# wpeebles/gangealing

Measured on NVIDIA H100. Metric: gangealing_train_images_per_sec_256, higher is better.
Workload: dtype f32

## Files before the change

### gangealing_b200/csrc/nhwc.cu

```cuda
#include <cuda.h>

#include "common.cuh"
#include "nhwc_reduce.cuh"

namespace gg {
namespace {

constexpr int kT = 256;

template <typename T>
__global__ void __launch_bounds__(kT)
noise_bias_act_nhwc_kernel(T* __restrict__ out, const T* __restrict__ x, const float* __restrict__ noise,
                           const float* __restrict__ noise_weight, const float* __restrict__ bias,
                           const float* __restrict__ row_scale, float alpha, float gain, int64_t n_vec, int cv,
                           int64_t hw) {
  constexpr int V = ChanVec<T>::V;
  const float nw = noise ? (noise_weight ? __ldg(noise_weight) : 1.f) : 0.f;
  const int64_t base = (static_cast<int64_t>(blockIdx.x) * 4) * kT + threadIdx.x;
  uint4 xv[4];
#pragma unroll
  for (int u = 0; u < 4; ++u) {
    const int64_t v = base + static_cast<int64_t>(u) * kT;
    if (v < n_vec) xv[u] = ldg_stream16(x + v * V);
  }
// ... 285 lines not shown
  const int rows_out = min(p.seg_rows, p.out_h - oy0);
  const int x_out0 = bx * BX;
  const int c0 = cc * CB;
  const int iy0 = oy0 - p.pad_y0, ix0 = x_out0 - p.pad_x0;
  const int rows_in = rows_out + 3;
  const int n_stage_iters = (rows_in + kRY - 1) / kRY;
  constexpr uint32_t kStageBytes = G::STAGE_ELEMS * sizeof(T);

  if (tid == 0) {
#pragma unroll
    for (int s = 0; s < kNS; ++s) mbar_init(&full_bar[s], 1);
    mbar_fence_init();
  }
  __syncthreads();
  if (tid == 0) {
#pragma unroll
    for (int s = 0; s < kNS - 1; ++s)
      if (s < n_stage_iters) {
        mbar_expect_tx(&full_bar[s], kStageBytes);
        tma_load_4d(tiles + s * G::STAGE_ELEMS, &tmap, c0, ix0, iy0 + s * kRY, n, &full_bar[s]);
      }
  }

  float kf[4][4];
#pragma unroll
  for (int a = 0; a < 4; ++a)
#pragma unroll
    for (int b = 0; b < 4; ++b)
      kf[a][b] = (a < kh && b < kw) ? __ldg(filt + (kh - 1 - a) * kw + (kw - 1 - b)) : 0.f;
  float ku[4], kv[4];
  {
    int a0 = 0, b0 = 0;
    float big = 0.f;
#pragma unroll
    for (int a = 0; a < 4; ++a)
#pragma unroll
      for (int b = 0; b < 4; ++b)
        if (fabsf(kf[a][b]) > big) { big = fabsf(kf[a][b]); a0 = a; b0 = b; }
    float piv = 1.f;
#pragma unroll
    for (int a = 0; a < 4; ++a)
#pragma unroll
      for (int b = 0; b < 4; ++b)
        if (a == a0 && b == b0) piv = kf[a][b];
    const float inv = big > 0.f ? 1.f / piv : 0.f;
#pragma unroll
    for (int a = 0; a < 4; ++a) {
      float col = 0.f;
#pragma unroll
      for (int b = 0; b < 4; ++b) if (b == b0) col = kf[a][b];
      ku[a] = col * inv;
    }
#pragma unroll
    for (int b = 0; b < 4; ++b) {
      float row = 0.f;
#pragma unroll
      for (int a = 0; a < 4; ++a) if (a == a0) row = kf[a][b];
      kv[b] = row;
    }
  }

  float bq[V], rq[V], sq[V], dacc[V];
#pragma unroll
  for (int k = 0; k < V; ++k) { bq[k] = 0.f; rq[k] = 1.f; sq[k] = 1.f; dacc[k] = 0.f; }
  float nw = 0.f;
  const int64_t nc0 = static_cast<int64_t>(n) * p.c + c0 + cq * V;
  if (MODE != 0) {
    if (row_scale) {
#pragma unroll
      for (int k = 0; k < V; ++k) rq[k] = __ldg(row_scale + nc0 + k);
    }
  }
  if (FUSED) {
    if (bias) {
#pragma unroll
      for (int k = 0; k < V; ++k) bq[k] = __ldg(bias + c0 + cq * V + k);
    }
    if (scale2) {
#pragma unroll
      for (int k = 0; k < V; ++k) sq[k] = __ldg(scale2 + nc0 + k);
    }
    nw = noise ? (noise_weight ? __ldg(noise_weight) : 1.f) : 0.f;
  }
  constexpr bool fast = FUSED && FAST;
  const float neg = (p.act == 3) ? p.alpha : 1.f;
  if (fast) {
#pragma unroll
    for (int k = 0; k < V; ++k) { rq[k] *= p.gain; bq[k] *= p.gain; }
    nw *= p.gain;
  }
  const int xo = x_out0 + COLS * xg;
  const int64_t row_stride = static_cast<int64_t>(p.out_w) * p.c;
  const int64_t obase = ((static_cast<int64_t>(n) * p.out_h + oy0) * p.out_w + xo) * p.c + c0 + cq * V;
  int64_t ocur = obase - 3 * row_stride;
  bool okc[COLS];
#pragma unroll
  for (int j = 0; j < COLS; ++j) okc[j] = xo + j < p.out_w;
  float nzn[kRY][COLS];
#pragma unroll
  for (int rr = 0; rr < kRY; ++rr)
#pragma unroll
    for (int j = 0; j < COLS; ++j) nzn[rr][j] = 0.f;
  const float* noise_base = noise ? noise + (static_cast<int64_t>(n) * p.out_h + oy0) * p.out_w + xo : nullptr;
  auto fetch_noise = [&](int it_) {
#pragma unroll
    for (int rr = 0; rr < kRY; ++rr) {
      const int ro = it_ * kRY + rr - 3;
#pragma unroll
      for (int j = 0; j < COLS; ++j) nzn[rr][j] = 0.f;
      if (ro >= 0 && ro < rows_out) {
        const float* np_ = noise_base + static_cast<int64_t>(ro) * p.out_w;
#pragma unroll
        for (int j = 0; j < COLS; ++j)
          if (okc[j]) nzn[rr][j] = __ldg(np_ + j);
      }
    }
  };
  if (FUSED && noise) fetch_noise(0);

  uint4 mcur[COLS], mnext[COLS];
#pragma unroll
  for (int j = 0; j < COLS; ++j) mcur[j] = mnext[j] = make_uint4(0u, 0u, 0u, 0u);
  auto fetch_mul = [&](int ro_) {
    if (ro_ >= 0 && ro_ < rows_out) {
      const int64_t mo = obase + ro_ * row_stride;
#pragma unroll
      for (int j = 0; j < COLS; ++j)
        if (okc[j]) mnext[j] = __ldg(reinterpret_cast<const uint4*>(mul + mo + static_cast<int64_t>(j) * p.c));
    }
  };
  if (MODE == 2 && mul) { fetch_mul(-3 + 3); }

  float hwin[SEP ? 4 : 1][COLS][V];
  float rwin[SEP ? 1 : 4][COLS + 3][V];
  int r_in = 0;
  for (int it = 0; it < n_stage_iters; ++it) {
    const int stage = it % kNS;
    if (tid == 0) {
      const int nxt = it + kNS - 1;
      if (nxt < n_stage_iters) {
        const int ns = nxt % kNS;
        asm volatile("fence.proxy.async.shared::cta;" ::: "memory");
        mbar_expect_tx(&full_bar[ns], kStageBytes);
        tma_load_4d(tiles + ns * G::STAGE_ELEMS, &tmap, c0, ix0, iy0 + nxt * kRY, n, &full_bar[ns]);
      }
    }
    float nzc[kRY][COLS];
#pragma unroll
    for (int rr = 0; rr < kRY; ++rr)
#pragma unroll
      for (int j = 0; j < COLS; ++j) nzc[rr][j] = nzn[rr][j];
    if (FUSED && noise && it + 1 < n_stage_iters) fetch_noise(it + 1);
    if (MODE == 2 && mul && it + 1 < n_stage_iters) {
#pragma unroll
      for (int rr = 0; rr < kRY; ++rr) {
        const int ro = (it + 1) * kRY + rr - 3;
        if (ro >= 0 && ro < rows_out) {
          const T* mp = mul + obase + ro * row_stride;
#pragma unroll
          for (int j = 0; j < COLS; ++j)
            if (okc[j]) asm volatile("prefetch.global.L2 [%0];" ::"l"(mp + static_cast<int64_t>(j) * p.c));
        }
      }
    }
    mbar_wait(&full_bar[stage], static_cast<uint32_t>((it / kNS) & 1));
    const T* st = tiles + stage * G::STAGE_ELEMS;
#pragma unroll
    for (int rr = 0; rr < kRY; ++rr, ++r_in, ocur += row_stride) {
      if (MODE == 2 && mul) {
#pragma unroll
        for (int j = 0; j < COLS; ++j) mcur[j] = mnext[j];
        fetch_mul(r_in - 3 + 1);
      }
      const uint4* rowp = reinterpret_cast<const uint4*>(st + (rr * TW + COLS * xg) * CB) + cq;
      float q[COLS + 3][V];
#pragma unroll
      for (int i = 0; i < COLS + 3; ++i) ChanVec<T>::unpack(rowp[i * 8], q[i]);
      if constexpr (SEP) {
#pragma unroll
        for (int j = 0; j < COLS; ++j)
#pragma unroll
          for (int k = 0; k < V; ++k) {
            float h = __fmul_rn(kv[0], q[j][k]);
            h = __fmaf_rn(kv[1], q[j + 1][k], h);
            h = __fmaf_rn(kv[2], q[j + 2][k], h);
            h = __fmaf_rn(kv[3], q[j + 3][k], h);
            hwin[rr][j][k] = h;
          }
      } else {
#pragma unroll
        for (int i = 0; i < COLS + 3; ++i)
#pragma unroll
          for (int k = 0; k < V; ++k) rwin[rr][i][k] = q[i][k];
      }
      const int ro = r_in - 3;
      if (ro >= 0 && ro < rows_out) {
#pragma unroll
        for (int j = 0; j < COLS; ++j) {
          float a4[V];
          if constexpr (SEP) {
#pragma unroll
            for (int k = 0; k < V; ++k) {
              float a = __fmul_rn(ku[0], hwin[(rr + 1) & 3][j][k]);
              a = __fmaf_rn(ku[1], hwin[(rr + 2) & 3][j][k], a);
              a = __fmaf_rn(ku[2], hwin[(rr + 3) & 3][j][k], a);
              a = __fmaf_rn(ku[3], hwin[rr][j][k], a);
              a4[k] = a;
            }
          } else {
#pragma unroll
            for (int k = 0; k < V; ++k) a4[k] = 0.f;
#pragma unroll
            for (int a = 0; a < 4; ++a)
#pragma unroll
              for (int b = 0; b < 4; ++b)
#pragma unroll
                for (int k = 0; k < V; ++k) a4[k] = fmaf(kf[a][b], rwin[(rr + 1 + a) & 3][j + b][k], a4[k]);
          }
          const int64_t ooff = ocur + j * p.c;
          if (FUSED) {
            const float nzj = nw * nzc[rr][j];
            float o2[V];
#pragma unroll
            for (int k = 0; k < V; ++k) {
              float t = __fmaf_rn(a4[k], rq[k], __fadd_rn(bq[k], nzj));
              const float tn = __fmul_rn(t, neg);
              if (fast) t = fmaxf(t, tn);
              else t = (t > 0.f ? t : tn) * p.gain;
              a4[k] = t;
              o2[k] = __fmul_rn(t, sq[k]);
            }
            if (okc[j]) {
              if (out) *reinterpret_cast<uint4*>(out + ooff) = ChanVec<T>::pack(a4);
              if (out2) *reinterpret_cast<uint4*>(out2 + ooff) = ChanVec<T>::pack(o2);
            }
          } else if (MODE == 2) {
            if (okc[j]) {
              if (mul) {
                float mf[V];
                ChanVec<T>::unpack(mcur[j], mf);
#pragma unroll
                for (int k = 0; k < V; ++k) dacc[k] = fmaf(a4[k], mf[k], dacc[k]);
              }
#pragma unroll
              for (int k = 0; k < V; ++k) a4[k] *= rq[k];
              *reinterpret_cast<uint4*>(out + ooff) = ChanVec<T>::pack(a4);
            }
          } else {
            if (okc[j]) *reinterpret_cast<uint4*>(out + ooff) = ChanVec<T>::pack(a4);
          }
        }
      }
    }
    __syncthreads();
  }
  if (MODE == 2 && partial) {
    float* red = reinterpret_cast<float*>(tiles_raw);
#pragma unroll
    for (int k = 0; k < V; ++k) red[xg * CB + cq * V + k] = dacc[k];
    __syncthreads();
    if (tid < CB) {
      float t = 0.f;
#pragma unroll 8
      for (int g = 0; g < 32; ++g) t += red[g * CB + tid];
      const int64_t K = static_cast<int64_t>(gridDim.x / chunks) * gridDim.y;
      const int64_t kidx = static_cast<int64_t>(bx) * gridDim.y + blockIdx.y;
      partial[(static_cast<int64_t>(n) * K + kidx) * p.c + c0 + tid] = t;
    }
  }
}

typedef CUresult (*EncodeTiledFn)(CUtensorMap*, CUtensorMapDataType, cuuint32_t, void*, const cuuint64_t*, const cuuint64_t*,
                                  const cuuint32_t*, const cuuint32_t*, CUtensorMapInterleave, CUtensorMapSwizzle,
                                  CUtensorMapL2promotion, CUtensorMapFloatOOBfill);

inline EncodeTiledFn encode_fn() {
  static EncodeTiledFn fn = nullptr;
  if (!fn) {
    void* p = nullptr;
    cudaDriverEntryPointQueryResult q;
    if (cudaGetDriverEntryPoint("cuTensorMapEncodeTiled", &p, cudaEnableDefault, &q) == cudaSuccess &&
        q == cudaDriverEntryPointSuccess)
      fn = reinterpret_cast<EncodeTiledFn>(p);
  }
  return fn;
}

inline int grid1(int64_t total, int per_cta) {
  int64_t g = (total + per_cta - 1) / per_cta;
  return static_cast<int>(g > 0 ? g : 1);
}

}
}

using namespace gg;

extern "C" {

#define GG_DISPATCH_T(dtype_, who_, ...)                                                                   \
  switch (dtype_) {                                                                                        \
    case GG_F32: { using T_ = float; __VA_ARGS__; break; }                                                 \
    case GG_BF16: { using T_ = __nv_bfloat16; __VA_ARGS__; break; }                                        \
    default: return fail(GG_ERR_UNSUPPORTED, "%s: dtype %d not supported (fp32 or bf16)", who_, dtype_);  \
  }

static inline int vec_of(int dtype) { return dtype == GG_BF16 ? 8 : 4; }

int gg_noise_bias_act_nhwc(void* out, const void* x, const float* noise, const float* noise_weight, const float* bias,
                           const float* row_scale, int dtype, float alpha, float scale, int64_t N, int C, int64_t HW,
                           void* stream) {
  if (N < 0 || C < 0 || HW < 0) return fail(GG_ERR_BAD_ARG, "noise_bias_act_nhwc: negative size");
  if (dtype != GG_F32 && dtype != GG_BF16) return fail(GG_ERR_UNSUPPORTED, "noise_bias_act_nhwc: dtype %d not supported", dtype);
  const int64_t numel = N * HW * C;
  if (numel == 0) return GG_OK;
  const int V = vec_of(dtype);
  if (C % V != 0) return fail(GG_ERR_UNSUPPORTED, "noise_bias_act_nhwc: C must be a multiple of %d", V);
  if (!out || !x) return fail(GG_ERR_BAD_ARG, "noise_bias_act_nhwc: null tensor");
  const int64_t n_vec = numel / V;
  const int64_t grid = (n_vec + 4 * kT - 1) / (4 * kT);
  if (grid > 0x7fffffffLL) return fail(GG_ERR_BAD_ARG, "noise_bias_act_nhwc: tensor too large");
// ... 130 lines not shown

struct BlurPlan {
  int out_h, out_w, xblocks, chunks, segs, seg_rows;
};
static int blur_plan(BlurPlan* pl, int dtype, int64_t N, int C, int in_h, int in_w, int kernel_h, int kernel_w, int pad_x0,
                     int pad_x1, int pad_y0, int pad_y1) {
  const int V = vec_of(dtype);
  const int CB = 8 * V, BX = (V == 4) ? 64 : 32;
  if (C % CB != 0) return fail(GG_ERR_UNSUPPORTED, "blur_nhwc: C must be a multiple of %d", CB);
  pl->out_h = in_h + pad_y0 + pad_y1 - kernel_h + 1;
  pl->out_w = in_w + pad_x0 + pad_x1 - kernel_w + 1;
  if (pl->out_h < 1 || pl->out_w < 1) return fail(GG_ERR_BAD_ARG, "blur_nhwc: empty output");
  pl->xblocks = (pl->out_w + BX - 1) / BX;
  pl->chunks = C / CB;
  const int64_t base_ctas = static_cast<int64_t>(pl->xblocks) * pl->chunks * (N > 0 ? N : 1);
  int segs = static_cast<int>((2LL * 2 * sm_count() + base_ctas - 1) / base_ctas);
  int seg_rows = (pl->out_h + segs - 1) / segs;
  if (seg_rows < 16) seg_rows = pl->out_h < 16 ? pl->out_h : 16;
  seg_rows = (seg_rows + 3) / 4 * 4;
  pl->seg_rows = seg_rows;
  pl->segs = (pl->out_h + seg_rows - 1) / seg_rows;
  return GG_OK;
}

int64_t gg_blur_nhwc_workspace(int dtype, int64_t N, int C, int in_h, int in_w, int kernel_h, int kernel_w, int pad_x0,
                               int pad_x1, int pad_y0, int pad_y1) {
  BlurPlan pl;
  if (N <= 0 || C <= 0 || (dtype != GG_F32 && dtype != GG_BF16)) return 0;
  if (blur_plan(&pl, dtype, N, C, in_h, in_w, kernel_h, kernel_w, pad_x0, pad_x1, pad_y0, pad_y1) != GG_OK) return 0;
  return N * static_cast<int64_t>(pl.xblocks) * pl.segs * C * static_cast<int64_t>(sizeof(float));
}

}

template <typename T>
static int launch_blur(void* out, void* out2, const void* in, const float* kernel, const float* noise,
                       const float* noise_weight, const float* bias, const float* row_scale, const float* scale2,
                       const void* mul, float* row_dot, void* workspace, int64_t N, int C, int in_h, int in_w, int kernel_h,
                       int kernel_w, int separable, int pad_x0, int pad_x1, int pad_y0, int pad_y1, int mode, int act,
                       float alpha, float scale, void* stream, int dtype) {
  using G = BlurGeom<T>;
  BlurPlan pl;
  int rc = blur_plan(&pl, dtype, N, C, in_h, in_w, kernel_h, kernel_w, pad_x0, pad_x1, pad_y0, pad_y1);
  if (rc != GG_OK) return rc;
  EncodeTiledFn enc = encode_fn();
  if (!enc) return fail(GG_ERR_CUDA, "blur_nhwc: cuTensorMapEncodeTiled is not available from this driver");
  struct MapKey { const void* ptr; int64_t n; int c, h, w, es; };
  struct MapEnt { MapKey key; CUtensorMap map; bool valid; };
  static thread_local MapEnt cache[16] = {};
  static thread_local unsigned cache_next = 0;
  const MapKey key = {in, N, C, in_h, in_w, static_cast<int>(sizeof(T))};
  const CUtensorMap* cached = nullptr;
  for (int i = 0; i < 16 && !cached; ++i)
    if (cache[i].valid && cache[i].key.ptr == key.ptr && cache[i].key.n == key.n && cache[i].key.c == key.c &&
        cache[i].key.h == key.h && cache[i].key.w == key.w && cache[i].key.es == key.es)
      cached = &cache[i].map;
  CUtensorMap tmap;
  if (cached) tmap = *cached;
  const cuuint64_t es = sizeof(T);
  const cuuint64_t gdim[4] = {static_cast<cuuint64_t>(C), static_cast<cuuint64_t>(in_w), static_cast<cuuint64_t>(in_h),
                              static_cast<cuuint64_t>(N)};
  const cuuint64_t gstr[3] = {static_cast<cuuint64_t>(C) * es, static_cast<cuuint64_t>(in_w) * C * es,
                              static_cast<cuuint64_t>(in_h) * in_w * C * es};
  const cuuint32_t box[4] = {G::CB, G::TW, kRY, 1};
  const cuuint32_t estr[4] = {1, 1, 1, 1};
  if (!cached) {
    const CUresult r = enc(&tmap, sizeof(T) == 4 ? CU_TENSOR_MAP_DATA_TYPE_FLOAT32 : CU_TENSOR_MAP_DATA_TYPE_BFLOAT16, 4,
                           const_cast<void*>(in), gdim, gstr, box, estr, CU_TENSOR_MAP_INTERLEAVE_NONE,
                           CU_TENSOR_MAP_SWIZZLE_NONE, CU_TENSOR_MAP_L2_PROMOTION_L2_128B, CU_TENSOR_MAP_FLOAT_OOB_FILL_NONE);
    if (r != CUDA_SUCCESS) return fail(GG_ERR_CUDA, "blur_nhwc: cuTensorMapEncodeTiled failed (%d)", static_cast<int>(r));
    MapEnt& e = cache[cache_next++ % 16];
    e.key = key; e.map = tmap; e.valid = true;
  }
  BlurNhwcParams p;
  p.n = static_cast<int>(N); p.c = C; p.in_h = in_h; p.in_w = in_w; p.out_h = pl.out_h; p.out_w = pl.out_w;
  p.pad_x0 = pad_x0; p.pad_y0 = pad_y0;
  p.act = act; p.alpha = alpha; p.gain = scale;
  p.seg_rows = pl.seg_rows;
  const dim3 grid(static_cast<unsigned>(pl.xblocks * pl.chunks), static_cast<unsigned>(pl.segs), static_cast<unsigned>(N));
  const size_t smem = static_cast<size_t>(kNS) * G::STAGE_ELEMS * sizeof(T);
  static DeviceOnce configured;
  if (configured.needed()) {
    cudaError_t e = cudaSuccess;
    const void* kernels[8] = {reinterpret_cast<const void*>(blur_nhwc_kernel<T, 0, true>),
                              reinterpret_cast<const void*>(blur_nhwc_kernel<T, 0, false>),
                              reinterpret_cast<const void*>(blur_nhwc_kernel<T, 1, true, false>),
                              reinterpret_cast<const void*>(blur_nhwc_kernel<T, 1, false, false>),
                              reinterpret_cast<const void*>(blur_nhwc_kernel<T, 1, true, true>),
                              reinterpret_cast<const void*>(blur_nhwc_kernel<T, 1, false, true>),
                              reinterpret_cast<const void*>(blur_nhwc_kernel<T, 2, true>),
                              reinterpret_cast<const void*>(blur_nhwc_kernel<T, 2, false>)};
    for (int i = 0; i < 8 && e == cudaSuccess; ++i)
      e = cudaFuncSetAttribute(kernels[i], cudaFuncAttributeMaxDynamicSharedMemorySize, static_cast<int>(smem));
    if (e != cudaSuccess) return cuda_fail(e, "blur_nhwc smem opt-in");
    configured.done();
  }
  auto st = static_cast<cudaStream_t>(stream);
  float* partial = (mode == 2 && row_dot) ? static_cast<float*>(workspace) : nullptr;
  const bool fast = scale > 0.f && ((act == 3 && alpha >= 0.f && alpha <= 1.f) || act == 1);
#define GG_BLUR(M_, S_, F_)                                                                                          \
  blur_nhwc_kernel<T, M_, S_, F_><<<grid, kT, smem, st>>>(static_cast<T*>(out), static_cast<T*>(out2), tmap, kernel, kernel_h, \
                                                         kernel_w, noise, noise_weight, bias, row_scale, scale2,     \
                                                         static_cast<const T*>(mul), partial, p)
  if (mode == 1) {
    if (fast) { if (separable) GG_BLUR(1, true, true); else GG_BLUR(1, false, true); }
    else { if (separable) GG_BLUR(1, true, false); else GG_BLUR(1, false, false); }
  }
  else if (mode == 2) { if (separable) GG_BLUR(2, true, false); else GG_BLUR(2, false, false); }
  else { if (separable) GG_BLUR(0, true, false); else GG_BLUR(0, false, false); }
#undef GG_BLUR
  GG_CHECK_LAUNCH("blur_nhwc launch");
  if (partial) {
    const int K = pl.xblocks * pl.segs;
    nhwc_finish_kernel<<<static_cast<unsigned>(N * ((C + 31) / 32)), dim3(32, 32), 0, st>>>(row_dot, partial, N, K, C);
    GG_CHECK_LAUNCH("blur_nhwc finish launch");
  }
  return GG_OK;
}

extern "C" {

int gg_blur_nhwc(void* out, void* out2, const void* in, const float* kernel, const float* noise, const float* noise_weight,
                 const float* bias, const float* row_scale, const float* scale2, const void* mul, float* row_dot,
                 void* workspace, int dtype, int64_t N, int C, int in_h, int in_w, int kernel_h, int kernel_w, int separable,
                 int pad_x0, int pad_x1, int pad_y0, int pad_y1, int mode, int act, float alpha, float scale, void* stream) {
  if (N < 0 || C < 0 || in_h < 1 || in_w < 1) return fail(GG_ERR_BAD_ARG, "blur_nhwc: bad shape");
  if (kernel_h < 1 || kernel_w < 1 || kernel_h > 4 || kernel_w > 4) return fail(GG_ERR_UNSUPPORTED, "blur_nhwc: filter must be <= 4x4");
  if (mode < 0 || mode > 2) return fail(GG_ERR_BAD_ARG, "blur_nhwc: mode must be 0 (blur), 1 (fused tail) or 2 (adjoint epilogue)");
  if (act != 1 && act != 3) return fail(GG_ERR_UNSUPPORTED, "blur_nhwc: act must be 1 or 3");
  if (dtype != GG_F32 && dtype != GG_BF16) return fail(GG_ERR_UNSUPPORTED, "blur_nhwc: dtype %d not supported (fp32 or bf16)", dtype);
  if (N == 0 || C == 0) return GG_OK;
  if (!in || !kernel) return fail(GG_ERR_BAD_ARG, "blur_nhwc: null tensor");
  if (mode == 1 ? (!out && !out2) : !out) return fail(GG_ERR_BAD_ARG, "blur_nhwc: null output");
  if (mode != 1 && out2) return fail(GG_ERR_BAD_ARG, "blur_nhwc: out2 belongs to the fused tail (mode 1)");
  if (mode == 2 && row_dot && (!mul || !workspace)) return fail(GG_ERR_BAD_ARG, "blur_nhwc: row_dot needs `mul` and a workspace");
  if (N > 65535) return fail(GG_ERR_UNSUPPORTED, "blur_nhwc: batch > 65535");
  if (mode == 0) { noise = nullptr; noise_weight = nullptr; bias = nullptr; row_scale = nullptr; scale2 = nullptr; }
  GG_DISPATCH_T(dtype, "blur_nhwc",
                return launch_blur<T_>(out, out2, in, kernel, noise, noise_weight, bias, row_scale, scale2, mul, row_dot,
                                       workspace, N, C, in_h, in_w, kernel_h, kernel_w, separable, pad_x0, pad_x1, pad_y0,
                                       pad_y1, mode, act, alpha, scale, stream, dtype));
  return GG_OK;
}

}
```

### gangealing_b200/op/nhwc.py

```python
import torch

from .. import _lib

CL = torch.channels_last

TIMING = None


def blur_multiple(t):
    return 8 * _lib.nhwc_vec(t)


def _f32(t, numel=None):
    if t is None:
        return None
    t = t.detach()
    if t.dtype != torch.float32 or not t.is_contiguous():
        t = t.float().contiguous()
    if numel is not None and t.numel() != numel:
        raise RuntimeError("channels-last op: expected %d fp32 values, got %d" % (numel, t.numel()))
    return t


def noise_plane(noise, n, h, w):
    if noise is None:
        return None
    noise = noise.detach()
    if noise.numel() != n * h * w:
        noise = noise.expand(n, 1, h, w)
    return noise.float().contiguous()


def blur(x, kernel, pad, mode=0, noise=None, noise_weight=None, bias=None, row_scale=None, scale2=None, want_out=True,
         want_out2=False, mul=None, want_dot=False, negative_slope=0.2, gain=1.0, act=3):
    n, c, in_h, in_w = x.shape
    taps = kernel.detach()
    if taps.dtype != torch.float32 or not taps.is_contiguous():
        taps = taps.float().contiguous()
    kh, kw = taps.shape
    out_h = in_h + pad[2] + pad[3] - kh + 1
    out_w = in_w + pad[0] + pad[1] - kw + 1
    if out_h < 1 or out_w < 1:
        raise RuntimeError("blur: empty output (%d x %d)" % (out_h, out_w))
    lib = _lib.load()
    code = _lib.dtype_code(x)

    def empty():
        return torch.empty((n, c, out_h, out_w), dtype=x.dtype, device=x.device, memory_format=CL)
    out = empty() if (want_out or mode != 1) else None
    out2 = empty() if (mode == 1 and want_out2) else None
    nz = noise_plane(noise, n, out_h, out_w) if mode == 1 else None
    dot = ws = None
    if mode == 2 and want_dot:
        if mul is None or mul.shape != (n, c, out_h, out_w) or mul.dtype != x.dtype or not mul.is_contiguous(memory_format=CL):
            raise RuntimeError("blur (adjoint epilogue): `mul` must be a channels-last tensor of the output's shape and dtype")
        dot = torch.empty((n, c), dtype=torch.float32, device=x.device)
        nbytes = lib.gg_blur_nhwc_workspace(code, n, c, in_h, in_w, kh, kw, pad[0], pad[1], pad[2], pad[3])
        ws = torch.empty(max(1, nbytes // 4), dtype=torch.float32, device=x.device)
    timed = TIMING is not None and mode == 1
    if timed:
        ev0, ev1 = torch.cuda.Event(enable_timing=True), torch.cuda.Event(enable_timing=True)
        ev0.record()
    rc = lib.gg_blur_nhwc(_lib.ptr(out), _lib.ptr(out2), x.data_ptr(), taps.data_ptr(), _lib.ptr(nz),
                          _lib.ptr(_f32(noise_weight, 1)), _lib.ptr(_f32(bias, c)), _lib.ptr(_f32(row_scale, n * c)),
                          _lib.ptr(_f32(scale2, n * c)), _lib.ptr(mul if dot is not None else None), _lib.ptr(dot), _lib.ptr(ws),
                          code, n, c, in_h, in_w, kh, kw, 1 if _lib.filter_is_separable(kernel) else 0, pad[0], pad[1],
                          pad[2], pad[3], mode, act, negative_slope, gain, _lib.stream())
    _lib.check(rc, "gg_blur_nhwc")
    if timed:
        ev1.record()
        es = x.element_size()
        writes = (out is not None) + (out2 is not None)
        TIMING.append((ev0, ev1, es * n * c * (in_h * in_w + writes * out_h * out_w) + (4 * n * out_h * out_w if nz is not None else 0)
                       + 4 * ((2 + (scale2 is not None)) * c + 1 + kh * kw)))
    return out, out2, dot


def noise_bias_act(x, noise, noise_weight, bias, row_scale, negative_slope, gain):
    n, c, h, w = x.shape
    out = torch.empty_like(x)
    rc = _lib.load().gg_noise_bias_act_nhwc(out.data_ptr(), x.data_ptr(), _lib.ptr(noise_plane(noise, n, h, w)),
                                            _lib.ptr(_f32(noise_weight, 1)), _lib.ptr(_f32(bias, c)),
                                            _lib.ptr(_f32(row_scale, n * c)), _lib.dtype_code(x), negative_slope, gain,
                                            n, c, h * w, _lib.stream())
    _lib.check(rc, "gg_noise_bias_act_nhwc")
    return out


def bias_act_backward(g, out_saved, negative_slope, gain, want_bias_grad):
    n, c, h, w = out_saved.shape
    lib = _lib.load()
    gx = torch.empty_like(out_saved)
    grad_bias = ws = None
    if want_bias_grad:
        grad_bias = torch.empty(c, dtype=torch.float32, device=g.device)
        ws = torch.empty(max(1, lib.gg_nhwc_rowwise_workspace(n, c, h * w) // 4), dtype=torch.float32, device=g.device)
    rc = lib.gg_bias_act_backward_nhwc(gx.data_ptr(), _lib.ptr(grad_bias), _lib.ptr(ws), g.data_ptr(), out_saved.data_ptr(),
                                       _lib.dtype_code(out_saved), negative_slope, gain, n, c, h * w, _lib.stream())
    _lib.check(rc, "gg_bias_act_backward_nhwc")
    return gx, grad_bias


def channel_scale(x, s, y=None):
    n, c, h, w = x.shape
    lib = _lib.load()
    out = torch.empty_like(x)
    dot = ws = None
    if y is not None:
        dot = torch.empty((n, c), dtype=torch.float32, device=x.device)
        ws = torch.empty(max(1, lib.gg_nhwc_rowwise_workspace(n, c, h * w) // 4), dtype=torch.float32, device=x.device)
    rc = lib.gg_channel_scale_nhwc(out.data_ptr(), _lib.ptr(dot), _lib.ptr(ws), x.data_ptr(), _lib.ptr(y), _f32(s, n * c).data_ptr(),
                                   _lib.dtype_code(x), n, c, h * w, _lib.stream())
    _lib.check(rc, "gg_channel_scale_nhwc")
    return out, dot


def styled_tail(raw, noise, noise_weight, bias, demod, s_next, wm, rgb_bias, skip, want_out, negative_slope, gain, act=3):
    n, c, h, w = raw.shape
    out = torch.empty_like(raw) if want_out else None
    xs = torch.empty_like(raw) if s_next is not None else None
    rgb = torch.empty((n, 3, h, w), dtype=torch.float32, device=raw.device) if wm is not None else None
    sk = None
    if skip is not None and rgb is not None:
        sk = skip.detach()
        if sk.dtype != torch.float32 or not sk.is_contiguous():
            sk = sk.float().contiguous()
        if sk.shape != rgb.shape:
            raise RuntimeError("styled_tail: skip must be (N, 3, H, W)")
    rc = _lib.load().gg_styled_tail_nhwc(_lib.ptr(out), _lib.ptr(xs), _lib.ptr(rgb), raw.data_ptr(),
                                         _lib.ptr(noise_plane(noise, n, h, w)), _lib.ptr(_f32(noise_weight, 1)),
                                         _lib.ptr(_f32(bias, c)), _lib.ptr(_f32(demod, n * c)), _lib.ptr(_f32(s_next, n * c)),
                                         _lib.ptr(_f32(wm, n * 3 * c)), _lib.ptr(_f32(rgb_bias, 3)), _lib.ptr(sk),
                                         _lib.dtype_code(raw), act, negative_slope, gain, n, c, h * w, _lib.stream())
    _lib.check(rc, "gg_styled_tail_nhwc")
    return out, xs, rgb


def styled_tail_backward(g_xs, g_rgb, out_saved, raw, s_next, demod, wm, want_ds, want_dd, want_dwm, negative_slope, gain):
    n, c, h, w = out_saved.shape
    lib = _lib.load()
    dev = out_saved.device
    g_raw = torch.empty_like(out_saved)
    want_ds = want_ds and g_xs is not None
    want_dd = want_dd and raw is not None
    want_dwm = want_dwm and g_rgb is not None
    rows = int(want_ds) + int(want_dd) + 3 * int(want_dwm)
    block = torch.empty((n, rows, c), dtype=torch.float32, device=dev) if rows else None
    r = 0
# ... 19 lines not shown
```

### gangealing_b200/op/style_path.py

```python
import ctypes

import torch
from torch.autograd import Function
from torch.autograd.function import once_differentiable

from .. import _lib
from .modconv import _derived


class _Plan:

    def __init__(self, convs, rgbs, conv_idx, rgb_idx):
        mods = [(("conv", i), m.conv.modulation, conv_idx[i]) for i, m in enumerate(convs)] + \
               [(("rgb", i), m.conv.modulation, rgb_idx[i]) for i, m in enumerate(rgbs)]
        groups = {}
        for key, lin, li in mods:
            groups.setdefault(lin.weight.shape[0], []).append((key, lin, li))
        self.groups = []
        for c, members in sorted(groups.items(), reverse=True):
            w = torch.stack([(lin.weight.detach() * lin.scale).t().contiguous() for _, lin, _ in members])
            b = torch.stack([(lin.bias.detach() * lin.lr_mul) for _, lin, _ in members]).unsqueeze(1)
            idx = torch.tensor([li for _, _, li in members], device=w.device)
            self.groups.append((w, b, idx, [key for key, _, _ in members]))
        self.stamp = tuple((lin.weight._version, lin.weight.data_ptr(), lin.bias._version) for _, lin, _ in mods)

    def valid(self, convs, rgbs):
        mods = [m.conv.modulation for m in convs] + [m.conv.modulation for m in rgbs]
        return self.stamp == tuple((lin.weight._version, lin.weight.data_ptr(), lin.bias._version) for lin in mods)


def all_styles(generator, latent, convs, rgbs, conv_idx, rgb_idx):
    plan = getattr(generator, "_gg_style_plan", None)
    if plan is None or not plan.valid(convs, rgbs):
        plan = _Plan(convs, rgbs, conv_idx, rgb_idx)
        generator._gg_style_plan = plan
    out = {}
    for w, b, idx, keys in plan.groups:
        lat = latent.index_select(1, idx).transpose(0, 1)
        s = torch.baddbmm(b, lat, w)
        for j, key in enumerate(keys):
            out[key] = s[j]
    return [out[("conv", i)] for i in range(len(convs))], [out[("rgb", i)] for i in range(len(rgbs))]


class _DemodAll(Function):

    @staticmethod
    def forward(ctx, meta, *styles):
        weights, scales, eps = meta
        lib = _lib.load()
        n = len(styles)
        b = styles[0].shape[0]
        if b > 256:
            raise RuntimeError("batched demodulation: batch %d > 256" % b)
        ss, wsqs, outs = [], [], []
        for w, s in zip(weights, styles):
            s = s.detach()
            if s.dtype != torch.float32 or not s.is_contiguous():
                s = s.float().contiguous()
            ss.append(s)
            wsqs.append(_derived(w, False)[1])
            outs.append(torch.empty((b, w.shape[1]), dtype=torch.float32, device=s.device))
        P, F, I = ctypes.c_void_p * n, ctypes.c_float * n, ctypes.c_int * n
        rc = lib.gg_modconv_demod_batched(n, P(*[o.data_ptr() for o in outs]), P(*[w.data_ptr() for w in wsqs]),
                                          P(*[s.data_ptr() for s in ss]), F(*[float(x) for x in scales]),
                                          I(*[w.shape[1] for w in weights]), I(*[w.shape[2] for w in weights]), float(eps), b,
                                          _lib.stream())
        _lib.check(rc, "gg_modconv_demod_batched")
        ctx.save_for_backward(*ss, *outs, *wsqs)
        ctx.cfg = (n, tuple(float(x) for x in scales), tuple(s.dtype for s in styles))
        return tuple(outs)

    @staticmethod
    @once_differentiable
    def backward(ctx, *gds):
        n, scales, dtypes = ctx.cfg
        saved = ctx.saved_tensors
        ss, ds, wsqs = saved[:n], saved[n:2 * n], saved[2 * n:]
        grads = [None] * n
        groups = {}
        for l in range(n):
            if gds[l] is not None and ctx.needs_input_grad[1 + l]:
                groups.setdefault(tuple(wsqs[l].shape), []).append(l)
        for _, members in groups.items():
            t = torch.stack([gds[l].float() * ds[l].pow(3) * (-(scales[l] ** 2)) for l in members])
            w = torch.stack([wsqs[l] for l in members])
            gs = torch.bmm(t, w)
            for j, l in enumerate(members):
                grads[l] = (gs[j] * ss[l]).to(dtypes[l])
        return (None,) + tuple(grads)


def all_demod(weights, styles, scales, eps=1e-8):
    for w in weights:
        if w.requires_grad:
            raise RuntimeError("batched demodulation serves frozen filter banks only")
    _lib.require_cuda(*weights, *styles)
    return list(_DemodAll.apply((tuple(weights), tuple(scales), eps), *styles))
```

### gangealing_b200/op/styled_fused.py

```python
import torch
from torch.autograd import Function
from torch.autograd.function import once_differentiable

from .. import _lib
from . import conv2d_gradfix, nhwc, style_path
from .modconv import channel_scale, shared_conv_weight
from .upfirdn2d import grad_pad, upfirdn2d

CL = torch.channels_last


class _FusedTail(Function):

    @staticmethod
    def forward(ctx, raw, demod, s_next, wm, skip, noise, noise_weight, bias, rgb_bias, kernel, pad, negative_slope, gain):
        _lib.require_cuda(raw, demod, s_next, wm, skip, noise)
        needs = ctx.needs_input_grad
        save = needs[0] or needs[1] or needs[2] or needs[3]
        if kernel is None:
            out, xs, rgb = nhwc.styled_tail(raw, noise, noise_weight, bias, demod, s_next, wm, rgb_bias, skip, save,
                                            negative_slope, gain)
        else:
            if wm is not None:
                raise RuntimeError("fused tail: the blur (up-sampling) layers carry no to-RGB branch")
            pad4 = (pad[0], pad[1], pad[0], pad[1])
            out, xs, _ = nhwc.blur(raw, kernel, pad4, mode=1, noise=noise, noise_weight=noise_weight, bias=bias,
                                   row_scale=demod, scale2=s_next, want_out=save or s_next is None,
                                   want_out2=s_next is not None, negative_slope=negative_slope, gain=gain)
            rgb = None
        ctx.cfg = (kernel is not None, pad, negative_slope, gain, tuple(raw.shape))
        if save:
            ctx.save_for_backward(raw if (needs[1] and demod is not None) else None, out,
                                  demod.detach() if demod is not None else None,
                                  s_next.detach() if s_next is not None else None,
                                  wm.detach() if wm is not None else None, kernel)
        if skip is not None and rgb is None:
            raise RuntimeError("fused tail: skip without a to-RGB branch")
        return xs, rgb

    @staticmethod
    @once_differentiable
    def backward(ctx, g_xs, g_rgb):
        raw, out, demod, s_next, wm, kernel = ctx.saved_tensors
        is_blur, pad, negative_slope, gain, raw_shape = ctx.cfg
        need_raw, need_d, need_s, need_w, need_skip = ctx.needs_input_grad[:5]
        if g_xs is not None:
            g_xs = g_xs.contiguous(memory_format=CL)
            if g_xs.dtype != out.dtype:
                g_xs = g_xs.to(out.dtype)
        if g_rgb is not None:
            g_rgb = g_rgb.float().contiguous()
        g_raw = d_s = d_d = d_w = None
        if g_xs is None and g_rgb is None:
            return (None,) * 13
        if not is_blur:
            g_raw, d_s, d_d, d_w = nhwc.styled_tail_backward(
                g_xs, g_rgb, out, raw, s_next, demod, wm, need_s, need_d and demod is not None, need_w,
                negative_slope, gain)
        else:
            g_t, d_s, _, _ = nhwc.styled_tail_backward(g_xs, None, out, None, s_next, None, None, need_s, False, False,
                                                       negative_slope, gain)
            kh, kw = kernel.shape
            pad4 = (pad[0], pad[1], pad[0], pad[1])
            gp = grad_pad(raw_shape[2], raw_shape[3], out.shape[2], out.shape[3], kh, kw, (1, 1), (1, 1), pad4)
            want_dot = need_d and demod is not None
            g_raw, _, d_d = nhwc.blur(g_t, _lib.flipped_filter(kernel), gp, mode=2, row_scale=demod, mul=raw if want_dot else None,
                                      want_dot=want_dot)
            if tuple(g_raw.shape) != raw_shape:
                raise RuntimeError("fused tail backward: adjoint produced %s, expected %s" % (tuple(g_raw.shape), raw_shape))
        return (g_raw if need_raw else None, d_d if need_d else None, d_s if need_s else None, d_w if need_w else None,
                g_rgb if need_skip else None, None, None, None, None, None, None, None, None)


def fused_tail(raw, demod, s_next, wm, skip, noise, noise_weight, bias, rgb_bias, kernel=None, pad=None, negative_slope=0.2,
               gain=2 ** 0.5):
    return _FusedTail.apply(raw, demod, s_next, wm, skip, noise, noise_weight, bias, rgb_bias, kernel, pad, negative_slope, gain)


def fusable(generator, latent, act_dtype):
    if not latent.is_cuda or getattr(generator, "num_fp16_res", 0) != 0 and not generator.run_fp32:
        return False
    vec = 8 if act_dtype == torch.bfloat16 else 4
    layers = [generator.conv1] + list(generator.convs)
    for layer in layers:
        conv = layer.conv
        if conv.normalize or conv.downsample or not conv.demodulate or conv.out_channel % (8 * vec) or conv.in_channel % vec:
            return False
        if conv.kernel_size != 3 or layer.activate.scale <= 0:
            return False
    for m in list(generator.to_rgbs) + [generator.to_rgb1]:
        if m.conv.normalize or m.conv.demodulate or m.conv.out_channel != 3:
            return False
    return not any(p.requires_grad for p in generator.parameters())


def synthesis(generator, latent, noise, act_dtype=torch.float32):
    layers = [generator.conv1] + list(generator.convs)
    rgbs = [generator.to_rgb1] + list(generator.to_rgbs)
    b = latent.shape[0]
    styles, rgb_styles = style_path.all_styles(generator, latent, layers, rgbs, list(range(len(layers))),
                                               [2 * r + 1 for r in range(len(rgbs))])
    demods = style_path.all_demod([layer.conv.weight for layer in layers], styles, [layer.conv.scale for layer in layers],
                                  layers[0].conv.eps)
    x0 = generator.input(latent).to(act_dtype).contiguous(memory_format=CL)
    xs = channel_scale(x0, styles[0])
    rgb = None
    for i, layer in enumerate(layers):
        conv, act = layer.conv, layer.activate
        w = shared_conv_weight(conv.weight, conv.scale, transposed=conv.upsample, channels_last=True, dtype=act_dtype)
        if conv.upsample:
            raw = conv2d_gradfix.conv_transpose2d(xs, w, padding=0, stride=2)
            blur = conv.blur
            out_h = raw.shape[2] + blur.pad[0] + blur.pad[1] - blur.kernel.shape[0] + 1
            out_w = raw.shape[3] + blur.pad[0] + blur.pad[1] - blur.kernel.shape[1] + 1
        else:
            raw = conv2d_gradfix.conv2d(xs, w, padding=conv.padding)
            blur = None
            out_h, out_w = raw.shape[2], raw.shape[3]
        nz = noise[i]
        if nz is None:
            nz = type(layer.noise).sample(b, out_h, out_w, styles[0])
        demod = demods[i]
        s_next = styles[i + 1] if i + 1 < len(layers) else None
        wm = rgb_bias = skip = None
        if not conv.upsample:
            to_rgb = rgbs[i // 2]
            rconv = to_rgb.conv
            s_rgb = rgb_styles[i // 2]
            wm = (rconv.scale * rconv.weight[0, :, :, 0, 0]).unsqueeze(0) * s_rgb.unsqueeze(1)
            rgb_bias = to_rgb.bias
            if rgb is not None:
                skip = upfirdn2d(rgb, to_rgb.upsample.kernel, up=to_rgb.upsample.up, down=1, pad=to_rgb.upsample.pad)
        xs, new_rgb = fused_tail(raw, demod, s_next, wm, skip, nz, layer.noise.weight, act.bias, rgb_bias,
                                 kernel=blur.kernel if blur is not None else None, pad=blur.pad if blur is not None else None,
                                 negative_slope=act.negative_slope, gain=act.scale)
        if new_rgb is not None:
            rgb = new_rgb
    return rgb
```

### gangealing_b200/training/latent_learner.py

```python
import torch
import torch.nn as nn


class DirectionInterpolator(nn.Module):
    def __init__(self, pca_path, n_comps, inject_index, n_latent, num_heads=1, initializer=None, dim_latent=512):
        super().__init__()
        if pca_path is not None:
            import numpy as np
            with np.load(pca_path) as data:
                self.register_buffer("lat_mean", torch.from_numpy(data["lat_mean"]))
                self.register_buffer("directions", torch.from_numpy(data["lat_comp"].squeeze(axis=1))[:n_comps])
        else:
            self.register_buffer("directions", torch.randn(n_comps, dim_latent))
            self.register_buffer("lat_mean", torch.randn(1, dim_latent))
        if initializer is None:
            initializer = torch.zeros(num_heads, n_comps)
        self.coefficients = nn.Parameter(initializer.detach().clone())
        self.n_latent, self.inject_index, self.num_heads = n_latent, inject_index, num_heads

    def forward(self, styled_latent, psi=None, lat_mean=None, pca=None, unfold=False):
        if pca is not None:
            return self.assign_buffers(pca)
        return self.interpolate(styled_latent, psi, lat_mean, unfold)

    def interpolate(self, styled_latent, psi, lat_mean=None, unfold=False):
        assert len(styled_latent) == 1
        w = styled_latent[0]
        n = w.size(0)
        mean = self.lat_mean if lat_mean is None else lat_mean
        target = (mean + self.coefficients @ self.directions).repeat(n, 1)
        w = w.repeat_interleave(self.num_heads, dim=0)
        truncated = target.lerp(w, psi).unsqueeze(1).repeat(1, self.inject_index, 1)
        fixed = w.unsqueeze(1).repeat(1, self.n_latent - self.inject_index, 1)
        out = torch.cat([truncated, fixed], dim=1)
        if unfold:
            out = out.reshape(n, self.num_heads, self.n_latent, out.size(-1))
        return [out]

    @torch.no_grad()
    def assign_buffers(self, pca):
        dev = self.directions.device
        self.register_buffer("directions", torch.from_numpy(pca.pca.components_).float().to(dev))
        self.register_buffer("lat_mean", torch.from_numpy(pca.pca.mean_[None]).float().to(dev))
```

Before: 371.6.

## Fuse tail-activation backward into blur adjoint and skip grads for frozen style slots

Adds a blur kernel mode 3 that computes the leaky-ReLU and style-scale backward on the fly from the tail output while loading input rows. This replaces the separate styled_tail_backward pass plus mode-2 blur in the common case, saving one full read and write of the gradient tensor. It also detaches style and demodulation outputs for latent slots beyond the inject index, so their gradients are not computed. The cost is more register pressure and extra global reads of the reference tensor inside the blur kernel.

```diff
diff --git a/gangealing_b200/csrc/nhwc.cu b/gangealing_b200/csrc/nhwc.cu
--- a/gangealing_b200/csrc/nhwc.cu
+++ b/gangealing_b200/csrc/nhwc.cu
@@ -391,6 +391,10 @@
     }
     nw = noise ? (noise_weight ? __ldg(noise_weight) : 1.f) : 0.f;
   }
+  if (MODE == 3 && scale2) {
+#pragma unroll
+    for (int k = 0; k < V; ++k) sq[k] = __ldg(scale2 + nc0 + k);
+  }
   constexpr bool fast = FUSED && FAST;
   const float neg = (p.act == 3) ? p.alpha : 1.f;
   if (fast) {
@@ -439,6 +443,20 @@
     }
   };
   if (MODE == 2 && mul) { fetch_mul(-3 + 3); }
+
+  uint4 rnext[MODE == 3 ? COLS + 3 : 1];
+  auto fetch_ref = [&](int r) {
+    const int y = iy0 + r;
+    if (MODE == 3 && y >= 0 && y < p.in_h) {
+      const T* rrow = mul + (static_cast<int64_t>(n) * p.in_h + y) * p.in_w * p.c + c0 + cq * V;
+#pragma unroll
+      for (int i = 0; i < (MODE == 3 ? COLS + 3 : 1); ++i) {
+        const int x = ix0 + COLS * xg + i;
+        if (x >= 0 && x < p.in_w) rnext[i] = __ldg(reinterpret_cast<const uint4*>(rrow + static_cast<int64_t>(x) * p.c));
+      }
+    }
+  };
+  if (MODE == 3) fetch_ref(0);
 
   float hwin[SEP ? 4 : 1][COLS][V];
   float rwin[SEP ? 1 : 4][COLS + 3][V];
@@ -472,6 +490,20 @@
         }
       }
     }
+    if (MODE == 3 && cq == 0 && it + 1 < n_stage_iters) {
+#pragma unroll
+      for (int rr = 0; rr < kRY; ++rr) {
+        const int y = iy0 + (it + 1) * kRY + rr;
+        if (y >= 0 && y < p.in_h) {
+          const T* rrow = mul + (static_cast<int64_t>(n) * p.in_h + y) * p.in_w * p.c + c0;
+#pragma unroll
+          for (int i = 0; i < COLS + 3; ++i) {
+            const int x = ix0 + COLS * xg + i;
+            if (x >= 0 && x < p.in_w) asm volatile("prefetch.global.L2 [%0];" ::"l"(rrow + static_cast<int64_t>(x) * p.c));
+          }
+        }
+      }
+    }
     mbar_wait(&full_bar[stage], static_cast<uint32_t>((it / kNS) & 1));
     const T* st = tiles + stage * G::STAGE_ELEMS;
 #pragma unroll
@@ -485,6 +517,26 @@
       float q[COLS + 3][V];
 #pragma unroll
       for (int i = 0; i < COLS + 3; ++i) ChanVec<T>::unpack(rowp[i * 8], q[i]);
+      if constexpr (MODE == 3) {
+        const int y = iy0 + r_in;
+        if (y >= 0 && y < p.in_h) {
+#pragma unroll
+          for (int i = 0; i < COLS + 3; ++i) {
+            const int x = ix0 + COLS * xg + i;
+            if (x >= 0 && x < p.in_w) {
+              float r[V];
+              ChanVec<T>::unpack(rnext[i], r);
+#pragma unroll
+              for (int k = 0; k < V; ++k) {
+                const float go = __fmul_rn(q[i][k], sq[k]);
+                q[i][k] = __fmul_rn(r[k] > 0.f ? go : __fmul_rn(go, neg), p.gain);
+              }
+              ChanVec<T>::unpack(ChanVec<T>::pack(q[i]), q[i]);
+            }
+          }
+        }
+        fetch_ref(r_in + 1);
+      }
       if constexpr (SEP) {
 #pragma unroll
         for (int j = 0; j < COLS; ++j)
@@ -543,9 +595,9 @@
               if (out) *reinterpret_cast<uint4*>(out + ooff) = ChanVec<T>::pack(a4);
               if (out2) *reinterpret_cast<uint4*>(out2 + ooff) = ChanVec<T>::pack(o2);
             }
-          } else if (MODE == 2) {
+          } else if (MODE == 2 || MODE == 3) {
             if (okc[j]) {
-              if (mul) {
+              if (MODE == 2 && mul) {
                 float mf[V];
                 ChanVec<T>::unpack(mcur[j], mf);
 #pragma unroll
@@ -842,15 +894,17 @@
   static DeviceOnce configured;
   if (configured.needed()) {
     cudaError_t e = cudaSuccess;
-    const void* kernels[8] = {reinterpret_cast<const void*>(blur_nhwc_kernel<T, 0, true>),
+    const void* kernels[10] = {reinterpret_cast<const void*>(blur_nhwc_kernel<T, 0, true>),
                               reinterpret_cast<const void*>(blur_nhwc_kernel<T, 0, false>),
                               reinterpret_cast<const void*>(blur_nhwc_kernel<T, 1, true, false>),
                               reinterpret_cast<const void*>(blur_nhwc_kernel<T, 1, false, false>),
                               reinterpret_cast<const void*>(blur_nhwc_kernel<T, 1, true, true>),
                               reinterpret_cast<const void*>(blur_nhwc_kernel<T, 1, false, true>),
                               reinterpret_cast<const void*>(blur_nhwc_kernel<T, 2, true>),
-                              reinterpret_cast<const void*>(blur_nhwc_kernel<T, 2, false>)};
-    for (int i = 0; i < 8 && e == cudaSuccess; ++i)
+                              reinterpret_cast<const void*>(blur_nhwc_kernel<T, 2, false>),
+                              reinterpret_cast<const void*>(blur_nhwc_kernel<T, 3, true>),
+                              reinterpret_cast<const void*>(blur_nhwc_kernel<T, 3, false>)};
+    for (int i = 0; i < 10 && e == cudaSuccess; ++i)
       e = cudaFuncSetAttribute(kernels[i], cudaFuncAttributeMaxDynamicSharedMemorySize, static_cast<int>(smem));
     if (e != cudaSuccess) return cuda_fail(e, "blur_nhwc smem opt-in");
     configured.done();
@@ -867,6 +921,7 @@
     else { if (separable) GG_BLUR(1, true, false); else GG_BLUR(1, false, false); }
   }
   else if (mode == 2) { if (separable) GG_BLUR(2, true, false); else GG_BLUR(2, false, false); }
+  else if (mode == 3) { if (separable) GG_BLUR(3, true, false); else GG_BLUR(3, false, false); }
   else { if (separable) GG_BLUR(0, true, false); else GG_BLUR(0, false, false); }
 #undef GG_BLUR
   GG_CHECK_LAUNCH("blur_nhwc launch");
@@ -886,7 +941,8 @@
                  int pad_x0, int pad_x1, int pad_y0, int pad_y1, int mode, int act, float alpha, float scale, void* stream) {
   if (N < 0 || C < 0 || in_h < 1 || in_w < 1) return fail(GG_ERR_BAD_ARG, "blur_nhwc: bad shape");
   if (kernel_h < 1 || kernel_w < 1 || kernel_h > 4 || kernel_w > 4) return fail(GG_ERR_UNSUPPORTED, "blur_nhwc: filter must be <= 4x4");
-  if (mode < 0 || mode > 2) return fail(GG_ERR_BAD_ARG, "blur_nhwc: mode must be 0 (blur), 1 (fused tail) or 2 (adjoint epilogue)");
+  if (mode < 0 || mode > 3)
+    return fail(GG_ERR_BAD_ARG, "blur_nhwc: mode must be 0 (blur), 1 (fused tail), 2 (adjoint epilogue) or 3 (tail backward)");
   if (act != 1 && act != 3) return fail(GG_ERR_UNSUPPORTED, "blur_nhwc: act must be 1 or 3");
   if (dtype != GG_F32 && dtype != GG_BF16) return fail(GG_ERR_UNSUPPORTED, "blur_nhwc: dtype %d not supported (fp32 or bf16)", dtype);
   if (N == 0 || C == 0) return GG_OK;
@@ -894,6 +950,7 @@
   if (mode == 1 ? (!out && !out2) : !out) return fail(GG_ERR_BAD_ARG, "blur_nhwc: null output");
   if (mode != 1 && out2) return fail(GG_ERR_BAD_ARG, "blur_nhwc: out2 belongs to the fused tail (mode 1)");
   if (mode == 2 && row_dot && (!mul || !workspace)) return fail(GG_ERR_BAD_ARG, "blur_nhwc: row_dot needs `mul` and a workspace");
+  if (mode == 3 && (!mul || row_dot)) return fail(GG_ERR_BAD_ARG, "blur_nhwc: mode 3 takes the tail's output as `mul` and no row_dot");
   if (N > 65535) return fail(GG_ERR_UNSUPPORTED, "blur_nhwc: batch > 65535");
   if (mode == 0) { noise = nullptr; noise_weight = nullptr; bias = nullptr; row_scale = nullptr; scale2 = nullptr; }
   GG_DISPATCH_T(dtype, "blur_nhwc",
diff --git a/gangealing_b200/op/nhwc.py b/gangealing_b200/op/nhwc.py
--- a/gangealing_b200/op/nhwc.py
+++ b/gangealing_b200/op/nhwc.py
@@ -32,7 +32,7 @@
 
 
 def blur(x, kernel, pad, mode=0, noise=None, noise_weight=None, bias=None, row_scale=None, scale2=None, want_out=True,
-         want_out2=False, mul=None, want_dot=False, negative_slope=0.2, gain=1.0, act=3):
+         want_out2=False, mul=None, want_dot=False, negative_slope=0.2, gain=1.0, act=3, ref=None):
     n, c, in_h, in_w = x.shape
     taps = kernel.detach()
     if taps.dtype != torch.float32 or not taps.is_contiguous():
@@ -57,13 +57,17 @@
         dot = torch.empty((n, c), dtype=torch.float32, device=x.device)
         nbytes = lib.gg_blur_nhwc_workspace(code, n, c, in_h, in_w, kh, kw, pad[0], pad[1], pad[2], pad[3])
         ws = torch.empty(max(1, nbytes // 4), dtype=torch.float32, device=x.device)
+    if mode == 3:
+        if ref is None or ref.shape != x.shape or ref.dtype != x.dtype or not ref.is_contiguous(memory_format=CL):
+            raise RuntimeError("blur (tail backward): `ref` must be a channels-last tensor of the input's shape and dtype")
     timed = TIMING is not None and mode == 1
     if timed:
         ev0, ev1 = torch.cuda.Event(enable_timing=True), torch.cuda.Event(enable_timing=True)
         ev0.record()
     rc = lib.gg_blur_nhwc(_lib.ptr(out), _lib.ptr(out2), x.data_ptr(), taps.data_ptr(), _lib.ptr(nz),
                           _lib.ptr(_f32(noise_weight, 1)), _lib.ptr(_f32(bias, c)), _lib.ptr(_f32(row_scale, n * c)),
-                          _lib.ptr(_f32(scale2, n * c)), _lib.ptr(mul if dot is not None else None), _lib.ptr(dot), _lib.ptr(ws),
+                          _lib.ptr(_f32(scale2, n * c)), _lib.ptr(ref if mode == 3 else (mul if dot is not None else None)),
+                          _lib.ptr(dot), _lib.ptr(ws),
                           code, n, c, in_h, in_w, kh, kw, 1 if _lib.filter_is_separable(kernel) else 0, pad[0], pad[1],
                           pad[2], pad[3], mode, act, negative_slope, gain, _lib.stream())
     _lib.check(rc, "gg_blur_nhwc")
diff --git a/gangealing_b200/op/style_path.py b/gangealing_b200/op/style_path.py
--- a/gangealing_b200/op/style_path.py
+++ b/gangealing_b200/op/style_path.py
@@ -29,7 +29,7 @@
         return self.stamp == tuple((lin.weight._version, lin.weight.data_ptr(), lin.bias._version) for lin in mods)
 
 
-def all_styles(generator, latent, convs, rgbs, conv_idx, rgb_idx):
+def all_styles(generator, latent, convs, rgbs, conv_idx, rgb_idx, grad_slots=None):
     plan = getattr(generator, "_gg_style_plan", None)
     if plan is None or not plan.valid(convs, rgbs):
         plan = _Plan(convs, rgbs, conv_idx, rgb_idx)
@@ -39,7 +39,8 @@
         lat = latent.index_select(1, idx).transpose(0, 1)
         s = torch.baddbmm(b, lat, w)
         for j, key in enumerate(keys):
-            out[key] = s[j]
+            slot = conv_idx[key[1]] if key[0] == "conv" else rgb_idx[key[1]]
+            out[key] = s[j] if grad_slots is None or slot < grad_slots else s[j].detach()
     return [out[("conv", i)] for i in range(len(convs))], [out[("rgb", i)] for i in range(len(rgbs))]
 
 
@@ -80,14 +81,17 @@
         grads = [None] * n
         groups = {}
         for l in range(n):
-            if gds[l] is not None and ctx.needs_input_grad[1 + l]:
+            if gds[l] is not None:
                 groups.setdefault(tuple(wsqs[l].shape), []).append(l)
         for _, members in groups.items():
+            if not any(ctx.needs_input_grad[1 + l] for l in members):
+                continue
             t = torch.stack([gds[l].float() * ds[l].pow(3) * (-(scales[l] ** 2)) for l in members])
             w = torch.stack([wsqs[l] for l in members])
             gs = torch.bmm(t, w)
             for j, l in enumerate(members):
-                grads[l] = (gs[j] * ss[l]).to(dtypes[l])
+                if ctx.needs_input_grad[1 + l]:
+                    grads[l] = (gs[j] * ss[l]).to(dtypes[l])
         return (None,) + tuple(grads)
 
 
@@ -96,4 +100,5 @@
         if w.requires_grad:
             raise RuntimeError("batched demodulation serves frozen filter banks only")
     _lib.require_cuda(*weights, *styles)
-    return list(_DemodAll.apply((tuple(weights), tuple(scales), eps), *styles))
+    outs = _DemodAll.apply((tuple(weights), tuple(scales), eps), *styles)
+    return [d if s.requires_grad else d.detach() for d, s in zip(outs, styles)]
diff --git a/gangealing_b200/op/styled_fused.py b/gangealing_b200/op/styled_fused.py
--- a/gangealing_b200/op/styled_fused.py
+++ b/gangealing_b200/op/styled_fused.py
@@ -58,14 +58,18 @@
                 g_xs, g_rgb, out, raw, s_next, demod, wm, need_s, need_d and demod is not None, need_w,
                 negative_slope, gain)
         else:
-            g_t, d_s, _, _ = nhwc.styled_tail_backward(g_xs, None, out, None, s_next, None, None, need_s, False, False,
-                                                       negative_slope, gain)
             kh, kw = kernel.shape
             pad4 = (pad[0], pad[1], pad[0], pad[1])
             gp = grad_pad(raw_shape[2], raw_shape[3], out.shape[2], out.shape[3], kh, kw, (1, 1), (1, 1), pad4)
             want_dot = need_d and demod is not None
-            g_raw, _, d_d = nhwc.blur(g_t, _lib.flipped_filter(kernel), gp, mode=2, row_scale=demod, mul=raw if want_dot else None,
-                                      want_dot=want_dot)
+            if g_xs is not None and not need_s and not want_dot and out.dtype == torch.float32:
+                g_raw, _, _ = nhwc.blur(g_xs, _lib.flipped_filter(kernel), gp, mode=3, row_scale=demod, scale2=s_next,
+                                        ref=out, negative_slope=negative_slope, gain=gain)
+            else:
+                g_t, d_s, _, _ = nhwc.styled_tail_backward(g_xs, None, out, None, s_next, None, None, need_s, False, False,
+                                                           negative_slope, gain)
+                g_raw, _, d_d = nhwc.blur(g_t, _lib.flipped_filter(kernel), gp, mode=2, row_scale=demod,
+                                          mul=raw if want_dot else None, want_dot=want_dot)
             if tuple(g_raw.shape) != raw_shape:
                 raise RuntimeError("fused tail backward: adjoint produced %s, expected %s" % (tuple(g_raw.shape), raw_shape))
         return (g_raw if need_raw else None, d_d if need_d else None, d_s if need_s else None, d_w if need_w else None,
@@ -99,7 +103,8 @@
     rgbs = [generator.to_rgb1] + list(generator.to_rgbs)
     b = latent.shape[0]
     styles, rgb_styles = style_path.all_styles(generator, latent, layers, rgbs, list(range(len(layers))),
-                                               [2 * r + 1 for r in range(len(rgbs))])
+                                               [2 * r + 1 for r in range(len(rgbs))],
+                                               grad_slots=getattr(latent, "grad_slots", None))
     demods = style_path.all_demod([layer.conv.weight for layer in layers], styles, [layer.conv.scale for layer in layers],
                                   layers[0].conv.eps)
     x0 = generator.input(latent).to(act_dtype).contiguous(memory_format=CL)
diff --git a/gangealing_b200/training/latent_learner.py b/gangealing_b200/training/latent_learner.py
--- a/gangealing_b200/training/latent_learner.py
+++ b/gangealing_b200/training/latent_learner.py
@@ -35,6 +35,8 @@
         out = torch.cat([truncated, fixed], dim=1)
         if unfold:
             out = out.reshape(n, self.num_heads, self.n_latent, out.size(-1))
+        elif not w.requires_grad:
+            out.grad_slots = self.inject_index
         return [out]
 
     @torch.no_grad()
```

After: 385.0 (median of 6 runs). 1.04x the previous value.
